# SGI-2022/Latent-Diffusion-Models-for-Shape-SDFs

Hardware: AMD Instinct MI355X
Metric: SDF queries/sec on 256^3 grid (+ DDPM sample steps/sec) (higher is better)
Workload: dtype bf16; 1 GPU; config4: decode B=64 shapes on a 256^3 grid on 1 rank (the whole grid is the one slab: no gather); batch=64, grid=256, latent_dim=256, decoder=DeepSDF 8x512 skip@4, parallelism=zslab1

## Files before the change

### latent-diffusion-models-for-shape-sdfs_amd/csrc/decoder_common.h

```cpp
#pragma once
#include "ldm_internal.h"

#include <math.h>

namespace ldm {
namespace dec {

enum DecMode { kModeGrid = 0, kModePoints = 1, kModeBricks = 2 };

#define LDM_STR2(x) #x
#define LDM_STR(x) LDM_STR2(x)

__device__ __forceinline__ float grid_axis(int i, float vs, float origin) {
#pragma clang fp contract(off)
    float t = (float)i * vs;
    return t + origin;
}

__device__ __forceinline__ void grid_point(int p, int N, int k0, float vs, float origin,
                                           float& x, float& y, float& z) {
    const int nn = N * N;
    const int k = k0 + p / nn;
    const int r = p - (p / nn) * nn;
    const int j = r / N;
    const int i = r - j * N;
    x = grid_axis(i, vs, origin);
    y = grid_axis(j, vs, origin);
    z = grid_axis(k, vs, origin);
}


template <typename T>
struct Elem;
template <>
struct Elem<__bf16> {
    static __device__ __forceinline__ unsigned pack(float a, float b) {
        typedef float f32x2 __attribute__((ext_vector_type(2)));
        const f32x2 v = {a, b};
        return __builtin_bit_cast(unsigned, __builtin_convertvector(v, bf16x2));
    }
    static __device__ __forceinline__ float round(float x) { return (float)(__bf16)x; }
    static __device__ __forceinline__ f32x16 mfma(u32x4 a, u32x4 b, f32x16 c) {
        return __builtin_amdgcn_mfma_f32_32x32x16_bf16(__builtin_bit_cast(bf16x8, a),
                                                       __builtin_bit_cast(bf16x8, b), c, 0, 0, 0);
    }
    static __device__ __forceinline__ f32x4 mfma16(u32x4 a, u32x4 b, f32x4 c) {
        return __builtin_amdgcn_mfma_f32_16x16x32_bf16(__builtin_bit_cast(bf16x8, a),
                                                       __builtin_bit_cast(bf16x8, b), c, 0, 0, 0);
    }
};
template <>
struct Elem<_Float16> {
    static __device__ __forceinline__ unsigned pack(float a, float b) {
        f16x2 v = {(_Float16)a, (_Float16)b};
        return __builtin_bit_cast(unsigned, v);
    }
    static __device__ __forceinline__ float round(float x) { return (float)(_Float16)x; }
    static __device__ __forceinline__ f32x16 mfma(u32x4 a, u32x4 b, f32x16 c) {
        return __builtin_amdgcn_mfma_f32_32x32x16_f16(__builtin_bit_cast(f16x8, a),
                                                      __builtin_bit_cast(f16x8, b), c, 0, 0, 0);
    }
    static __device__ __forceinline__ f32x4 mfma16(u32x4 a, u32x4 b, f32x4 c) {
        return __builtin_amdgcn_mfma_f32_16x16x32_f16(__builtin_bit_cast(f16x8, a),
                                                      __builtin_bit_cast(f16x8, b), c, 0, 0, 0);
    }
};


__device__ __forceinline__ unsigned relu2(unsigned v) {
    typedef short s16x2 __attribute__((ext_vector_type(2)));
    s16x2 x = __builtin_bit_cast(s16x2, v);
    const s16x2 z = {0, 0};
    x = __builtin_elementwise_max(x, z);
    return __builtin_bit_cast(unsigned, x);
}

template <typename T>
__device__ __forceinline__ void acc_to_frags(const f32x16& a, u32x4& f0, u32x4& f1) {
#pragma unroll
    for (int q = 0; q < 4; ++q) {
        f0[q] = relu2(Elem<T>::pack(a[2 * q], a[2 * q + 1]));
        f1[q] = relu2(Elem<T>::pack(a[8 + 2 * q], a[8 + 2 * q + 1]));
    }
}

}
}
```

### latent-diffusion-models-for-shape-sdfs_amd/csrc/decoder_fs.hip

```cpp
#include "decoder_common.h"

namespace ldm {
namespace {
using namespace dec;

constexpr int kFsD = 4;

constexpr int kFsStep = 2048;
constexpr int kFsAct = 33 * 4 * 1024;
constexpr int kFsRed = 4 * 4 * 64 * 4;
constexpr int kFsWl = 512 * 4;
#ifndef FS_STAMP
#define FS_STAMP 0
#endif
constexpr int kFsStamp = FS_STAMP ? 128 * 8 : 0;
#ifndef FS_ABL
#define FS_ABL 0
#endif
static_assert(FS_ABL == 0 || FS_STAMP, "ablations are diagnostic builds");
constexpr int kFsLds = kFsAct + kFsRed + kFsWl + kFsStamp;
static_assert(kFsLds <= 160 * 1024, "LDS");

__host__ __device__ constexpr int fs_nparts(int S) { return S == 256 ? 15 : 16; }
__host__ __device__ constexpr int fs_nsteps(int S) { return S == 256 ? 384 : 448; }

template <typename T>
__global__ void fs_aux_pack_kernel(const float* __restrict__ beta, const float* __restrict__ wxyz,
                                   int B, T* __restrict__ aux) {
    const int id = blockIdx.x * blockDim.x + threadIdx.x;
    if (id >= B * 4 * 4 * 2 * 64) return;
    const int lane = id & 63;
    const int i = (id >> 6) & 1;
    const int slot = (id >> 7) & 3;
    const int w = (id >> 9) & 3;
    const int b = id >> 11;
    const int li = slot >> 1;
    const int p = slot & 1;
    float v[8] = {0, 0, 0, 0, 0, 0, 0, 0};
    if (lane < 32) {
        const int f = 128 * w + 64 * p + 32 * i + lane;
        const float* wx = wxyz + ((size_t)li * kHidden + f) * 3;
        const float bb = beta[((size_t)b * 2 + li) * kHidden + f];
        const float hi = Elem<T>::round(bb);
        v[0] = wx[0]; v[1] = wx[1]; v[2] = wx[2];
        v[3] = wx[0]; v[4] = wx[1]; v[5] = wx[2];
        v[6] = hi;    v[7] = bb - hi;
    }
    T* o = aux + (size_t)id * 8;
#pragma unroll
    for (int e = 0; e < 8; ++e) o[e] = (T)v[e];
}

struct FArgs {
    const uint8_t* stream;
    const uint8_t* aux;
    const float* w_last;
    const float* xyz;
    float* out;
    float b_last;
    int npts, tiles_per_shape, n_tiles;
    int N, k0;
    float vs, origin;
    const int32_t* bricks;
    const int32_t* count;
    int nb, nbt;
};

enum FsEpi { FE_NONE = 0, FE_LATE = 1, FE_EARLY = 2, FE_FIN0 = 3, FE_FIN1 = 4 };

struct FSrc {
    bool shape;
    uint32_t off;
    bool none = false;
};

struct FCtx {
    int lane, wave, h;
    uint32_t voff;
    char* smem;
    __amdgpu_buffer_rsrc_t rw;
    __amdgpu_buffer_rsrc_t ra;
    uint32_t s_beg, s_end;
    uint32_t s_iss;
    uint32_t baux_w;
    uint32_t aux_w;
    uint32_t aux_next;
    u32x4 auxn[2];
    u32x4 ring[kFsD][2];
    u32x4 b[4];
    float part[4];
    float* out;
    int npts, prev_shape, prev_local;
    float b_last;
    unsigned long long* st;
    int st_i;
    bool st_on;
    const int32_t* bricks;
    int N, nb, nbt;
};

__device__ __forceinline__ void stamp(FCtx& c) {
    if (FS_STAMP) {
        if (c.st_on && c.lane == 0 && c.st_i < 128) c.st[c.st_i] = __builtin_readcyclecounter();
        ++c.st_i;
    }
}

__device__ __forceinline__ u32x4 bld(__amdgpu_buffer_rsrc_t r, uint32_t voff, uint32_t soff) {
    return __builtin_bit_cast(u32x4, __builtin_amdgcn_raw_buffer_load_b128(r, voff, soff, 0));
}

__device__ __forceinline__ void load_aux(FCtx& c, FSrc s) {
    if (s.none) return;
    const __amdgpu_buffer_rsrc_t r = s.shape ? c.ra : c.rw;
    c.auxn[0] = bld(r, c.voff, s.off);
    c.auxn[1] = bld(r, c.voff + 1024u, s.off);
}

__device__ __forceinline__ uint32_t opaque(uint32_t v) {
    asm volatile("" : "+v"(v));
    return v;
}

__device__ __forceinline__ int opaque_s(int v) {
    asm volatile("" : "+s"(v));
    return v;
}

__device__ __forceinline__ char* lds_at(const FCtx& c, uint32_t off) {
    return c.smem + (opaque(c.voff) + off);
}
__device__ __forceinline__ u32x4* act_w(const FCtx& c, int late) {
    return reinterpret_cast<u32x4*>(lds_at(c, (uint32_t)(late + 4 * c.wave) * 4096u));
}
__device__ __forceinline__ const f32x4* wl_at(const FCtx& c, int p, int i) {
    const uint32_t h = opaque(c.voff) >> 9;
    return reinterpret_cast<const f32x4*>(
        c.smem + kFsAct + kFsRed + (((c.wave * 2 + p) * 2 + i) * 2) * 64 + h * 64);
}

__device__ __forceinline__ float* red_w(const FCtx& c) {
    return reinterpret_cast<float*>(c.smem + kFsAct + c.wave * 4 * 64 * 4 + (opaque(c.voff) >> 2));
}

__device__ __forceinline__ void fs_bar() {
    if (FS_ABL & 4) return;
    asm volatile("s_waitcnt lgkmcnt(0)\n\ts_barrier" ::: "memory");
}

__device__ __forceinline__ void read_b(FCtx& c, int pos) {
    const u32x4* p = reinterpret_cast<const u32x4*>(lds_at(c, pos * 4096));
#pragma unroll
    for (int n = 0; n < 4; ++n) c.b[n] = p[n * 64];
}

__device__ __forceinline__ void issue(FCtx& c, int r) {
    const uint32_t so = c.s_iss + (uint32_t)(r >> 1) * 2u * kFsStep;
    const uint32_t vo = c.voff + (uint32_t)(r & 1) * kFsStep;
    if (FS_ABL & 1) return;
    c.ring[r][0] = bld(c.rw, vo, so);
    c.ring[r][1] = bld(c.rw, vo + 1024u, so);
}

__device__ __forceinline__ void next_group(FCtx& c) {
    c.s_iss += 4u * kFsStep;
    if (c.s_iss == c.s_end) c.s_iss = c.s_beg;
}

__device__ __forceinline__ float relu_f(float x) {
    return __builtin_bit_cast(float, max(__builtin_bit_cast(int, x), 0));
}

template <typename T, int EK>
__device__ __forceinline__ void epi_unit(FCtx& c, const f32x16 (&accY)[2][4], int u) {
    const int t = u >> 1, s = u & 1;
    const int i = t >> 2, n = t & 3;
    if (FS_ABL & 2) return;
    if (EK == FE_LATE || EK == FE_EARLY) {
        u32x4 f;
#pragma unroll
        for (int q = 0; q < 4; ++q)
            f[q] = relu2(Elem<T>::pack(accY[i][n][8 * s + 2 * q], accY[i][n][8 * s + 2 * q + 1]));
        u32x4* p = act_w(c, EK == FE_LATE ? 16 : 0);
        p[((2 * i + s) * 4 + n) * 64] = f;
    } else if (EK == FE_FIN0 || EK == FE_FIN1) {
        const f32x4* w = wl_at(c, EK == FE_FIN0 ? 0 : 1, i);
        float part = c.part[n];
#pragma unroll
        for (int q = 2 * s; q < 2 * s + 2; ++q) {
            const f32x4 wv = w[q];
#pragma unroll
            for (int e = 0; e < 4; ++e) part = fmaf(relu_f(accY[i][n][4 * q + e]), wv[e], part);
        }
        c.part[n] = part;
    }
}

template <typename T, int EK>
__device__ __forceinline__ void epi_step(FCtx& c, const f32x16 (&accY)[2][4], int k) {
    if (EK == FE_NONE || k == 15) return;
    epi_unit<T, EK>(c, accY, k);
    if (k == 14) epi_unit<T, EK>(c, accY, 15);
    if (EK == FE_FIN1 && k == 14) {
        float* rw = red_w(c);
#pragma unroll
        for (int n = 0; n < 4; ++n) {
            rw[n * 64] = c.part[n];
            c.part[n] = 0.f;
        }
    }
}

__device__ __forceinline__ void fin_store(const FCtx& c, int shape, int local) {
    const int lane = (int)(opaque(c.voff) >> 4);
    if (local < 0 || lane >= 32) return;
    const float* rr = reinterpret_cast<const float*>(
        c.smem + kFsAct + c.wave * 64 * 4 + (opaque(c.voff) >> 2));
    float s = 0.f;
#pragma unroll
    for (int w = 0; w < 4; ++w) s += rr[w * 4 * 64] + rr[w * 4 * 64 + 32];
    const int pt = local * kTilePoints + 32 * c.wave + lane;
    if (pt < c.npts) {
        const __amdgpu_buffer_rsrc_t ro = __builtin_amdgcn_make_buffer_rsrc(
            (void*)(c.out + (size_t)shape * c.npts), (short)0, 0x7ffffff0, 0x00020000);
        __builtin_amdgcn_raw_buffer_store_b32(__builtin_bit_cast(uint32_t, tanhf(s + c.b_last)),
                                              ro, (uint32_t)pt * 4u, 0, 2 );
    }
}

__device__ __forceinline__ int list_at(const int32_t* list, int i) {
    typedef const __attribute__((address_space(4))) int32_t* const_i32;
    return ((const_i32)(uintptr_t)list)[i];
}

__device__ __forceinline__ void brick_origin(int gid, int nb_, int& shape, int& i0, int& j0,
                                             int& k0) {
    const int nb = opaque_s(nb_);
    const int nb2 = nb * nb, nb3 = nb2 * nb;
    shape = gid / nb3;
    const int id = gid - shape * nb3;
    const int bz = id / nb2, r = id - bz * nb2;
    const int by = r / nb;
    i0 = 8 * (r - by * nb);
    j0 = 8 * by;
    k0 = 8 * bz;
}

__device__ __forceinline__ void fin_store_bricks(const FCtx& c, int tile) {
    const int lane = (int)(opaque(c.voff) >> 4);
    if (tile < 0 || lane >= 32) return;
    const float* rr = reinterpret_cast<const float*>(
        c.smem + kFsAct + c.wave * 64 * 4 + (opaque(c.voff) >> 2));
    float s = 0.f;
#pragma unroll
    for (int w = 0; w < 4; ++w) s += rr[w * 4 * 64] + rr[w * 4 * 64 + 32];
    const int gid = list_at(c.bricks, tile >> 2);
    LDM_DASSERT(gid >= 0 && gid < c.nbt);
    int shape, i0, j0, k0;
    brick_origin(gid, c.nb, shape, i0, j0, k0);
    const int idx = 128 * (tile & 3) + 32 * c.wave + lane;
    const int i = i0 + (idx & 7), j = j0 + ((idx >> 3) & 7);
    const int k = k0 + 2 * (tile & 3) + (c.wave >> 1);
    const int N = c.N;
    if ((unsigned)gid < (unsigned)c.nbt && i < N && j < N && k < N) {
        const __amdgpu_buffer_rsrc_t ro = __builtin_amdgcn_make_buffer_rsrc(
            (void*)(c.out + ((size_t)shape * N + k) * N * N), (short)0, 0x7ffffff0, 0x00020000);
        __builtin_amdgcn_raw_buffer_store_b32(__builtin_bit_cast(uint32_t, tanhf(s + c.b_last)),
                                              ro, (uint32_t)(j * N + i) * 4u, 0, 2 );
    }
}

template <int MODE>
__device__ __forceinline__ void fin_store_mode(const FCtx& c) {
    if (MODE == kModeBricks) fin_store_bricks(c, c.prev_local);
    else fin_store(c, c.prev_shape, c.prev_local);
}

__device__ __forceinline__ void valu_slot(int v) {
    if (v == 2) __builtin_amdgcn_sched_group_barrier(0x002, 2, 0);
    else if (v == 4) __builtin_amdgcn_sched_group_barrier(0x002, 4, 0);
}

template <typename T>
__device__ __forceinline__ void mfma_pair(f32x16 (&acc)[2][4], const u32x4& a0, const u32x4& a1,
                                          const u32x4& b, int n) {
    acc[0][n] = Elem<T>::mfma(a0, b, acc[0][n]);
    acc[1][n] = Elem<T>::mfma(a1, b, acc[1][n]);
}

template <typename T, int EK, int K0, int BAR>
__device__ __forceinline__ void group4(FCtx& c, f32x16 (&acc)[2][4], const f32x16 (&accY)[2][4],
                                       int p0) {
    constexpr int BP = 1;
    const char* gbase = lds_at(c, (p0 + 1) * 4096);
#pragma unroll
    for (int r = 0; r < 4; ++r) {
        const u32x4* nb = reinterpret_cast<const u32x4*>(gbase + r * 4096);
        const u32x4 a0 = c.ring[r][0], a1 = c.ring[r][1];
        const int k = K0 + r;
        const int V = (EK == FE_NONE || k == 15) ? 0 : (k == 14 ? 4 : 2);
        if (r == BAR) {
#pragma unroll
            for (int n = 0; n < BP; ++n) mfma_pair<T>(acc, a0, a1, c.b[n], n);
            for (int n = 0; n < BP; ++n) {
                __builtin_amdgcn_sched_group_barrier(0x008, 2, 0);
            }
            __builtin_amdgcn_sched_barrier(0);
            fs_bar();
            __builtin_amdgcn_sched_barrier(0);
#pragma unroll
            for (int n = 0; n < BP; ++n) c.b[n] = nb[n * 64];
#pragma unroll
            for (int n = BP; n < 4; ++n) {
                mfma_pair<T>(acc, a0, a1, c.b[n], n);
                c.b[n] = nb[n * 64];
            }
            issue(c, r);
            epi_step<T, EK>(c, accY, k);
            for (int n = 0; n < BP; ++n) __builtin_amdgcn_sched_group_barrier(0x100, 1, 0);
            for (int n = BP; n < 4; ++n) {
                __builtin_amdgcn_sched_group_barrier(0x008, 1, 0);
                valu_slot(V);
                __builtin_amdgcn_sched_group_barrier(0x008, 1, 0);
                __builtin_amdgcn_sched_group_barrier(0x100, 1, 0);
                valu_slot(V);
            }
        } else {
#pragma unroll
            for (int n = 0; n < 4; ++n) {
                mfma_pair<T>(acc, a0, a1, c.b[n], n);
                c.b[n] = nb[n * 64];
            }
            issue(c, r);
            epi_step<T, EK>(c, accY, k);
#pragma unroll
            for (int n = 0; n < 4; ++n) {
                __builtin_amdgcn_sched_group_barrier(0x008, 1, 0);
                valu_slot(V);
                __builtin_amdgcn_sched_group_barrier(0x008, 1, 0);
                __builtin_amdgcn_sched_group_barrier(0x100, 1, 0);
                valu_slot(V);
            }
        }
        __builtin_amdgcn_sched_group_barrier(0x020, 2, 0);
        __builtin_amdgcn_sched_barrier(0);
    }
    next_group(c);
}

template <typename T, int EK, bool BAR>
__device__ __forceinline__ void steps16e(FCtx& c, f32x16 (&acc)[2][4],
                                         const f32x16 (&accY)[2][4], int p0) {
    group4<T, EK, 0, -1>(c, acc, accY, p0);
    group4<T, EK, 4, -1>(c, acc, accY, p0 + 4);
    group4<T, EK, 8, -1>(c, acc, accY, p0 + 8);
    group4<T, EK, 12, BAR ? 3 : -1>(c, acc, accY, p0 + 12);
}

template <typename T>
__device__ __forceinline__ void steps_plain(FCtx& c, f32x16 (&acc)[2][4],
                                            const f32x16 (&accY)[2][4], int pos0, int j0, int j1) {
#pragma unroll 1
    for (int j = j0; j < j1; j += 4) group4<T, FE_NONE, 0, -1>(c, acc, accY, pos0 + j);
}

template <typename T, int EK, bool E16, int MODE = kModeGrid>
__device__ __forceinline__ void run_part(FCtx& c, f32x16 (&acc)[2][4], const f32x16 (&accY)[2][4],
                                         int nk, bool mid, bool endbar, FSrc naux, int pos0,
                                         bool bar0) {
    const f32x16 zero = {};
    const u32x4 a0 = c.auxn[0], a1 = c.auxn[1];
    if (nk == 0) {
#pragma unroll
        for (int n = 0; n < 4; ++n) {
            acc[0][n] = Elem<T>::mfma(a0, c.b[n], zero);
            acc[1][n] = Elem<T>::mfma(a1, c.b[n], zero);
        }
        load_aux(c, naux);
        stamp(c);
        return;
    }
    if (bar0) {
#pragma unroll
        for (int n = 0; n < 4; ++n) {
            acc[0][n] = Elem<T>::mfma(a0, c.b[n], zero);
            acc[1][n] = Elem<T>::mfma(a1, c.b[n], zero);
        }
        load_aux(c, naux);
        fs_bar();
        read_b(c, pos0);
    } else {
        const u32x4* p = reinterpret_cast<const u32x4*>(lds_at(c, pos0 * 4096));
#pragma unroll
        for (int n = 0; n < 4; ++n) {
            acc[0][n] = Elem<T>::mfma(a0, c.b[n], zero);
            acc[1][n] = Elem<T>::mfma(a1, c.b[n], zero);
            c.b[n] = p[n * 64];
        }
        load_aux(c, naux);
#pragma unroll
        for (int n = 0; n < 4; ++n) {
            __builtin_amdgcn_sched_group_barrier(0x008, 2, 0);
            __builtin_amdgcn_sched_group_barrier(0x100, 1, 0);
        }
        __builtin_amdgcn_sched_group_barrier(0x020, 2, 0);
        __builtin_amdgcn_sched_barrier(0);
    }
    stamp(c);
    if (!E16 && EK != FE_NONE) {
        if (mid || (endbar && nk == 16)) steps16e<T, EK, true>(c, acc, accY, pos0);
        else steps16e<T, EK, false>(c, acc, accY, pos0);
        if (EK == FE_FIN1) fin_store_mode<MODE>(c);
        stamp(c);
        if (endbar && nk == 32) {
            steps_plain<T>(c, acc, accY, pos0, 16, 28);
            group4<T, FE_NONE, 0, 3>(c, acc, accY, pos0 + 28);
        } else {
            steps_plain<T>(c, acc, accY, pos0, 16, nk);
        }
    } else if (E16) {
        steps_plain<T>(c, acc, accY, pos0, 0, 12);
        group4<T, FE_NONE, 0, 3>(c, acc, accY, pos0 + 12);
        stamp(c);
        if (endbar) steps16e<T, EK, true>(c, acc, accY, pos0 + 16);
        else steps16e<T, EK, false>(c, acc, accY, pos0 + 16);
    } else {
        steps_plain<T>(c, acc, accY, pos0, 0, nk < 16 ? nk : 16);
        stamp(c);
        steps_plain<T>(c, acc, accY, pos0, 16, nk);
    }
    stamp(c);
}

template <typename T, bool LATE>
__device__ __forceinline__ void acc_to_lds(FCtx& c, const f32x16 (&acc)[2][4]) {
    u32x4* p = act_w(c, LATE ? 16 : 0);
#pragma unroll
    for (int i = 0; i < 2; ++i)
#pragma unroll
        for (int n = 0; n < 4; ++n) {
            u32x4 f0, f1;
            acc_to_frags<T>(acc[i][n], f0, f1);
            p[(2 * i * 4 + n) * 64] = f0;
            p[((2 * i + 1) * 4 + n) * 64] = f1;
        }
}

template <typename T, int S, int MODE>
__global__ __launch_bounds__(256, 1) void dec_fs_kernel(FArgs a) {
    __shared__ __attribute__((aligned(16))) char smem[kFsLds];
    FCtx c;
    c.lane = threadIdx.x & 63;
    c.wave = __builtin_amdgcn_readfirstlane(threadIdx.x >> 6);
    c.h = c.lane >> 5;
    c.voff = (uint32_t)c.lane * 16u;
    c.smem = smem;
    c.out = a.out;
    c.npts = a.npts;
    c.b_last = a.b_last;
    c.prev_shape = 0;
    c.prev_local = -1;
    c.st = reinterpret_cast<unsigned long long*>(smem + kFsAct + kFsRed + kFsWl);
    c.st_i = 0;
    c.st_on = false;
    float* wl = reinterpret_cast<float*>(smem + kFsAct + kFsRed);

    for (int i = threadIdx.x; i < 512; i += 256) wl[i] = a.w_last[i];
    __syncthreads();
    const int n_tiles = MODE == kModeBricks ? 4 * min(max(a.count[0], 0), a.nbt) : a.n_tiles;
    if (MODE == kModeBricks) {
        c.bricks = a.bricks;
        c.N = a.N;
        c.nb = a.nb;
        c.nbt = a.nbt;
    }
    if ((int)blockIdx.x >= n_tiles) return;

    constexpr int NST = fs_nsteps(S);
    constexpr int NP = fs_nparts(S);
    constexpr uint32_t kFlags = 0x00020000u;
    c.rw = __builtin_amdgcn_make_buffer_rsrc((void*)a.stream, (short)0, 0x7ffffff0, kFlags);
    c.ra = __builtin_amdgcn_make_buffer_rsrc((void*)a.aux, (short)0, 0x7ffffff0, kFlags);
    c.s_beg = (uint32_t)c.wave * NST * kFsStep;
    c.s_end = c.s_beg + NST * kFsStep;
    c.s_iss = c.s_beg;
    c.baux_w = (uint32_t)(4 * NST + c.wave * NP) * kFsStep;
    auto brick_of = [&](int tile) -> int {
        return min(max(list_at(a.bricks, tile >> 2), 0), a.nbt - 1);
    };
    auto shape_aux = [&](int tile) -> uint32_t {
        if (MODE == kModeBricks) {
            const int nb = opaque_s(a.nb);
            return ((uint32_t)(brick_of(tile) / (nb * nb * nb)) * 4u + (uint32_t)c.wave) * 4u *
                   kFsStep;
        }
        return ((uint32_t)(tile / a.tiles_per_shape) * 4u + (uint32_t)c.wave) * 4u * kFsStep;
    };
    auto bias = [&](int pi) -> FSrc { return FSrc{false, c.baux_w + (uint32_t)pi * kFsStep}; };
    auto shp = [&](int slot) -> FSrc { return FSrc{true, c.aux_w + (uint32_t)slot * kFsStep}; };
    c.aux_w = shape_aux(blockIdx.x);
#pragma unroll
    for (int r = 0; r < kFsD; ++r) issue(c, r);
    next_group(c);

    f32x16 accA[2][4], accB[2][4];
#pragma unroll
    for (int i = 0; i < 2; ++i)
#pragma unroll
        for (int n = 0; n < 4; ++n) accB[i][n] = f32x16{};
#pragma unroll
    for (int n = 0; n < 4; ++n) c.part[n] = 0.f;
#pragma unroll 1
    for (int tile = blockIdx.x; tile < n_tiles; tile += gridDim.x) {
        int shape, local, bi0 = 0, bj0 = 0, bk0 = 0;
        if (MODE == kModeBricks) {
            brick_origin(brick_of(tile), a.nb, shape, bi0, bj0, bk0);
            local = tile;
        } else {
            shape = tile / a.tiles_per_shape;
            local = tile - shape * a.tiles_per_shape;
        }
        {
            const int nt = tile + (int)gridDim.x;
            c.aux_next = nt < n_tiles ? shape_aux(nt) : c.aux_w;
        }
        c.st_on = FS_STAMP && c.wave == 0 && tile == (int)blockIdx.x + (int)gridDim.x;
        c.st_i = 0;
        stamp(c);
        load_aux(c, shp(0));
        const uint32_t lv = opaque(c.voff);
        const bool hi = lv >= 512u;
#pragma unroll
        for (int n = 0; n < 4; ++n) {
            int pt = local * kTilePoints + 32 * n + (int)((lv >> 4) & 31u);
            if (pt >= a.npts) pt = a.npts - 1;
            float x, y, z;
            if (MODE == kModeBricks) {
                const int idx = 128 * (tile & 3) + 32 * n + (int)((lv >> 4) & 31u);
                const int m = a.N - 1;
                x = grid_axis(min(bi0 + (idx & 7), m), a.vs, a.origin);
                y = grid_axis(min(bj0 + ((idx >> 3) & 7), m), a.vs, a.origin);
                z = grid_axis(min(bk0 + (idx >> 6), m), a.vs, a.origin);
            } else if (MODE == kModePoints) {
                const float* qq = a.xyz + ((size_t)shape * a.npts + pt) * 3;
                x = qq[0];
                y = qq[1];
                z = qq[2];
            } else {
                grid_point(pt, opaque_s(a.N), a.k0, a.vs, a.origin, x, y, z);
            }
            const float xh = Elem<T>::round(x), yh = Elem<T>::round(y), zh = Elem<T>::round(z);
            u32x4 f;
            f[0] = hi ? 0u : Elem<T>::pack(xh, yh);
            f[1] = hi ? 0u : Elem<T>::pack(zh, x - xh);
            f[2] = hi ? 0u : Elem<T>::pack(y - yh, z - zh);
            f[3] = hi ? 0u : Elem<T>::pack(1.f, 1.f);
            reinterpret_cast<u32x4*>(lds_at(c, 32u * 4096u))[n * 64] = f;
        }
        read_b(c, 32);

        run_part<T, FE_NONE, false>(c, accA, accB, 0, false, false, shp(1), 0, false);
        acc_to_lds<T, false>(c, accA);
        stamp(c);
        run_part<T, FE_NONE, false>(c, accA, accB, 0, false, false, bias(2), 0, false);
        acc_to_lds<T, true>(c, accA);
        stamp(c);

        int pi = 2;
        run_part<T, FE_FIN1, false, MODE>(c, accA, accB, 32, true, false, bias(pi + 1), 0, true);
        run_part<T, FE_EARLY, true>(c, accB, accA, 32, true, true, bias(pi + 2), 0, false);
        pi += 2;
        constexpr int L2P = S == 256 ? 3 : 4;
#pragma unroll 1
        for (int l = 2; l < L2P; ++l, pi += 2) {
            const FSrc nx = (S == 512 && l == 3) ? shp(2) : bias(pi + 2);
            run_part<T, FE_LATE, false>(c, accA, accB, 32, true, false, bias(pi + 1), 0, false);
            run_part<T, FE_EARLY, true>(c, accB, accA, 32, true, true, nx, 0, false);
        }
        if (S == 256) {
            run_part<T, FE_LATE, false>(c, accA, accB, 32, true, false, shp(2), 0, false);
            fs_bar();
            acc_to_lds<T, true>(c, accA);
            stamp(c);
            run_part<T, FE_NONE, false>(c, accA, accB, 16, false, false, shp(3), 16, true);
            run_part<T, FE_EARLY, false>(c, accB, accA, 16, false, true, bias(pi + 3), 16,
                                             false);
            pi += 3;
        } else {
            run_part<T, FE_LATE, false>(c, accA, accB, 32, true, false, shp(3), 0, false);
            run_part<T, FE_EARLY, true>(c, accB, accA, 32, true, true, bias(pi + 2), 0, false);
            pi += 2;
        }
#pragma unroll 1
        for (int l = 5; l < 7; ++l, pi += 2) {
            run_part<T, FE_LATE, false>(c, accA, accB, 32, true, false, bias(pi + 1), 0, false);
            run_part<T, FE_EARLY, true>(c, accB, accA, 32, true, true, bias(pi + 2), 0, false);
        }
        run_part<T, FE_LATE, false>(c, accA, accB, 32, true, false, bias(pi + 1), 0, false);
        run_part<T, FE_FIN0, false>(c, accB, accA, 32, false, true, FSrc{true, 0, true}, 0,
                                        false);
        c.prev_shape = shape;
        c.prev_local = local;
        c.aux_w = c.aux_next;
    }
#pragma unroll
    for (int u = 0; u < 16; ++u) epi_unit<T, FE_FIN1>(c, accB, u);
    {
        float* rw = red_w(c);
#pragma unroll
        for (int n = 0; n < 4; ++n) rw[n * 64] = c.part[n];
    }
    fs_bar();
    fin_store_mode<MODE>(c);
    asm volatile("s_waitcnt vmcnt(0)" ::: "memory");
    if (FS_STAMP && c.wave == 0) {
        __builtin_amdgcn_s_waitcnt(0);
        for (int k = c.lane; k < 128; k += 64)
            reinterpret_cast<unsigned long long*>(a.out)[(size_t)blockIdx.x * 128 + k] = c.st[k];
    }
}

template <typename T, int S>
void launch_fs(const FArgs& a, bool points, hipStream_t s, int grid) {
    if (points)
        hipLaunchKernelGGL((dec_fs_kernel<T, S, kModePoints>), dim3(grid), dim3(256), 0, s, a);
    else
        hipLaunchKernelGGL((dec_fs_kernel<T, S, kModeGrid>), dim3(grid), dim3(256), 0, s, a);
}

template <typename T, int S>
void launch_fs_bricks(const FArgs& a, hipStream_t s, int grid) {
    hipLaunchKernelGGL((dec_fs_kernel<T, S, kModeBricks>), dim3(grid), dim3(256), 0, s, a);
}

}

size_t decoder_fs_aux_bytes(int B) { return (size_t)B * 4 * 4 * kFsStep; }

int decoder_fs_n_stages(int skip_width) { return fs_nsteps(skip_width == 253 ? 256 : 512); }

int decoder_fs_fwd(const ldm_decoder_t* w, const float* beta, const float* xyz, int B, int npts,
                   int N, int k0, float vs, float origin, float* out, void* ws, size_t ws_bytes,
                   hipStream_t s, int num_cus, const int32_t* bricks, const int32_t* count,
                   int n_bricks) {
    const int S = w->skip_width == 253 ? 256 : 512;
    LDM_REQUIRE(w->n_stages == fs_nsteps(S), LDM_EINVAL, "split layout: n_stages %d != %d",
                w->n_stages, fs_nsteps(S));
    LDM_REQUIRE(ws != nullptr && ws_bytes >= decoder_fs_aux_bytes(B) && LDM_ALIGNED(ws, 16),
                LDM_ENOSPC, "workspace too small: need %zu bytes, got %zu",
                decoder_fs_aux_bytes(B), ws_bytes);
    LDM_REQUIRE((size_t)B * 4 * 4 * kFsStep < 0x7ffffff0u, LDM_EINVAL,
                "split layout: %d shapes exceed the aux buffer range", B);
    {
        const int n = B * 4 * 4 * 2 * 64;
        if (w->dtype == LDM_BF16)
            hipLaunchKernelGGL(fs_aux_pack_kernel<__bf16>, dim3((n + 255) / 256), dim3(256), 0, s,
                               beta, w->wxyz, B, (__bf16*)ws);
        else
            hipLaunchKernelGGL(fs_aux_pack_kernel<_Float16>, dim3((n + 255) / 256), dim3(256), 0,
                               s, beta, w->wxyz, B, (_Float16*)ws);
        if (int e = launch_status("fs_aux_pack")) return e;
    }
    FArgs a;
    a.stream = (const uint8_t*)w->weights;
    a.aux = (const uint8_t*)ws;
    a.w_last = w->w_last;
    a.xyz = xyz;
    a.out = out;
    a.b_last = w->b_last;
    a.npts = npts;
    a.tiles_per_shape = (npts + kTilePoints - 1) / kTilePoints;
    a.n_tiles = B * a.tiles_per_shape;
    a.bricks = bricks;
    a.count = count;
    a.nb = (N + 7) / 8;
    a.nbt = n_bricks;
    const int mode = bricks ? kModeBricks : xyz ? kModePoints : kModeGrid;
    if (mode == kModeBricks) a.n_tiles = 4 * n_bricks;
    a.N = N;
    a.k0 = k0;
    a.vs = vs;
    a.origin = origin;
    const int grid = a.n_tiles < num_cus ? a.n_tiles : num_cus;
    if (mode != kModeBricks) {
        const bool points = mode == kModePoints;
        if (w->dtype == LDM_BF16) {
            if (S == 256) launch_fs<__bf16, 256>(a, points, s, grid);
            else launch_fs<__bf16, 512>(a, points, s, grid);
        } else {
            if (S == 256) launch_fs<_Float16, 256>(a, points, s, grid);
            else launch_fs<_Float16, 512>(a, points, s, grid);
        }
    } else if (w->dtype == LDM_BF16) {
        if (S == 256) launch_fs_bricks<__bf16, 256>(a, s, grid);
        else launch_fs_bricks<__bf16, 512>(a, s, grid);
    } else {
        if (S == 256) launch_fs_bricks<_Float16, 256>(a, s, grid);
        else launch_fs_bricks<_Float16, 512>(a, s, grid);
    }
    return launch_status("ldm_decoder_fwd(split)");
}

}
```

Before: 471.3 million queries/s.

## Pipeline layer-0 MFMAs with LDS stores and cheapen grid index division

```diff
diff --git a/latent-diffusion-models-for-shape-sdfs_amd/csrc/decoder_common.h b/latent-diffusion-models-for-shape-sdfs_amd/csrc/decoder_common.h
--- a/latent-diffusion-models-for-shape-sdfs_amd/csrc/decoder_common.h
+++ b/latent-diffusion-models-for-shape-sdfs_amd/csrc/decoder_common.h
@@ -1,4 +1,5 @@
 #pragma once
+#include "grid_index.h"
 #include "ldm_internal.h"
 
 #include <math.h>
@@ -44,6 +45,11 @@
         return __builtin_amdgcn_mfma_f32_32x32x16_bf16(__builtin_bit_cast(bf16x8, a),
                                                        __builtin_bit_cast(bf16x8, b), c, 0, 0, 0);
     }
+    static __device__ __forceinline__ f32x16 mfma_v(u32x4 a, u32x4 b) {
+        f32x16 d;
+        asm volatile("v_mfma_f32_32x32x16_bf16 %0, %1, %2, 0" : "=&v"(d) : "v"(a), "v"(b));
+        return d;
+    }
     static __device__ __forceinline__ f32x4 mfma16(u32x4 a, u32x4 b, f32x4 c) {
         return __builtin_amdgcn_mfma_f32_16x16x32_bf16(__builtin_bit_cast(bf16x8, a),
                                                        __builtin_bit_cast(bf16x8, b), c, 0, 0, 0);
@@ -59,6 +65,11 @@
     static __device__ __forceinline__ f32x16 mfma(u32x4 a, u32x4 b, f32x16 c) {
         return __builtin_amdgcn_mfma_f32_32x32x16_f16(__builtin_bit_cast(f16x8, a),
                                                       __builtin_bit_cast(f16x8, b), c, 0, 0, 0);
+    }
+    static __device__ __forceinline__ f32x16 mfma_v(u32x4 a, u32x4 b) {
+        f32x16 d;
+        asm volatile("v_mfma_f32_32x32x16_f16 %0, %1, %2, 0" : "=&v"(d) : "v"(a), "v"(b));
+        return d;
     }
     static __device__ __forceinline__ f32x4 mfma16(u32x4 a, u32x4 b, f32x4 c) {
         return __builtin_amdgcn_mfma_f32_16x16x32_f16(__builtin_bit_cast(f16x8, a),
diff --git a/latent-diffusion-models-for-shape-sdfs_amd/csrc/decoder_fs.hip b/latent-diffusion-models-for-shape-sdfs_amd/csrc/decoder_fs.hip
--- a/latent-diffusion-models-for-shape-sdfs_amd/csrc/decoder_fs.hip
+++ b/latent-diffusion-models-for-shape-sdfs_amd/csrc/decoder_fs.hip
@@ -64,6 +64,7 @@
     const int32_t* bricks;
     const int32_t* count;
     int nb, nbt;
+    GridDiv gd;
 };
 
 enum FsEpi { FE_NONE = 0, FE_LATE = 1, FE_EARLY = 2, FE_FIN0 = 3, FE_FIN1 = 4 };
@@ -171,6 +172,11 @@
     return __builtin_bit_cast(float, max(__builtin_bit_cast(int, x), 0));
 }
 
+__device__ __forceinline__ float acc_read(float a) {
+    asm volatile("" : "+a"(a));
+    return a;
+}
+
 template <typename T, int EK>
 __device__ __forceinline__ void epi_unit(FCtx& c, const f32x16 (&accY)[2][4], int u) {
     const int t = u >> 1, s = u & 1;
@@ -190,7 +196,11 @@
         for (int q = 2 * s; q < 2 * s + 2; ++q) {
             const f32x4 wv = w[q];
 #pragma unroll
-            for (int e = 0; e < 4; ++e) part = fmaf(relu_f(accY[i][n][4 * q + e]), wv[e], part);
+            for (int e = 0; e < 4; ++e) {
+                const float v = EK == FE_FIN1 ? acc_read(accY[i][n][4 * q + e])
+                                              : accY[i][n][4 * q + e];
+                part = fmaf(relu_f(v), wv[e], part);
+            }
         }
         c.part[n] = part;
     }
@@ -370,16 +380,6 @@
                                          bool bar0) {
     const f32x16 zero = {};
     const u32x4 a0 = c.auxn[0], a1 = c.auxn[1];
-    if (nk == 0) {
-#pragma unroll
-        for (int n = 0; n < 4; ++n) {
-            acc[0][n] = Elem<T>::mfma(a0, c.b[n], zero);
-            acc[1][n] = Elem<T>::mfma(a1, c.b[n], zero);
-        }
-        load_aux(c, naux);
-        stamp(c);
-        return;
-    }
     if (bar0) {
 #pragma unroll
         for (int n = 0; n < 4; ++n) {
@@ -410,7 +410,10 @@
     if (!E16 && EK != FE_NONE) {
         if (mid || (endbar && nk == 16)) steps16e<T, EK, true>(c, acc, accY, pos0);
         else steps16e<T, EK, false>(c, acc, accY, pos0);
-        if (EK == FE_FIN1) fin_store_mode<MODE>(c);
+        if (EK == FE_FIN1) {
+            stamp(c);
+            fin_store_mode<MODE>(c);
+        }
         stamp(c);
         if (endbar && nk == 32) {
             steps_plain<T>(c, acc, accY, pos0, 16, 28);
@@ -432,9 +435,9 @@
     stamp(c);
 }
 
-template <typename T, bool LATE>
+template <typename T>
 __device__ __forceinline__ void acc_to_lds(FCtx& c, const f32x16 (&acc)[2][4]) {
-    u32x4* p = act_w(c, LATE ? 16 : 0);
+    u32x4* p = act_w(c, 16);
 #pragma unroll
     for (int i = 0; i < 2; ++i)
 #pragma unroll
@@ -444,6 +447,31 @@
             p[(2 * i * 4 + n) * 64] = f0;
             p[((2 * i + 1) * 4 + n) * 64] = f1;
         }
+}
+
+template <typename T, bool LATE>
+__device__ __forceinline__ void layer0_part(FCtx& c, FSrc naux) {
+    const u32x4 a[2] = {c.auxn[0], c.auxn[1]};
+    u32x4* p = act_w(c, LATE ? 16 : 0);
+    f32x16 t[2];
+    t[0] = Elem<T>::mfma_v(a[0], c.b[0]);
+#pragma unroll
+    for (int q = 0; q < 8; ++q) {
+        const int i = q & 1, n = q >> 1;
+        if (q < 7) t[(q + 1) & 1] = Elem<T>::mfma_v(a[(q + 1) & 1], c.b[(q + 1) >> 1]);
+        if (q == 0) {
+            asm volatile("s_nop 10" : "+v"(t[0]));
+            load_aux(c, naux);
+            stamp(c);
+        }
+        __builtin_amdgcn_sched_barrier(0);
+        u32x4 f0, f1;
+        acc_to_frags<T>(t[q & 1], f0, f1);
+        p[(2 * i * 4 + n) * 64] = f0;
+        p[((2 * i + 1) * 4 + n) * 64] = f1;
+        __builtin_amdgcn_sched_barrier(0);
+    }
+    stamp(c);
 }
 
 template <typename T, int S, int MODE>
@@ -530,6 +558,17 @@
         load_aux(c, shp(0));
         const uint32_t lv = opaque(c.voff);
         const bool hi = lv >= 512u;
+        const uint32_t p0 = (uint32_t)local * kTilePoints;
+        uint32_t ti = 0, tj = 0, tk = 0;
+        if (MODE == kModeGrid) {
+            grid_first(p0, (uint32_t)a.N, a.gd, ti, tj, tk);
+            tk += (uint32_t)a.k0;
+        }
+        const float* row = nullptr;
+        if (MODE == kModePoints) {
+            row = a.xyz + (size_t)shape * a.npts * 3;
+            asm volatile("" : "+s"(row));
+        }
 #pragma unroll
         for (int n = 0; n < 4; ++n) {
             int pt = local * kTilePoints + 32 * n + (int)((lv >> 4) & 31u);
@@ -542,12 +581,18 @@
                 y = grid_axis(min(bj0 + ((idx >> 3) & 7), m), a.vs, a.origin);
                 z = grid_axis(min(bk0 + (idx >> 6), m), a.vs, a.origin);
             } else if (MODE == kModePoints) {
-                const float* qq = a.xyz + ((size_t)shape * a.npts + pt) * 3;
+                const float* qq = row + (size_t)pt * 3;
                 x = qq[0];
                 y = qq[1];
                 z = qq[2];
             } else {
-                grid_point(pt, opaque_s(a.N), a.k0, a.vs, a.origin, x, y, z);
+                const uint32_t off =
+                    grid_tail_off(p0, 32u * n + ((lv >> 4) & 31u), (uint32_t)a.npts);
+                uint32_t vi, vj, vk;
+                grid_voxel(ti, tj, tk, off, (uint32_t)a.N, a.gd.m, vi, vj, vk);
+                x = grid_axis((int)vi, a.vs, a.origin);
+                y = grid_axis((int)vj, a.vs, a.origin);
+                z = grid_axis((int)vk, a.vs, a.origin);
             }
             const float xh = Elem<T>::round(x), yh = Elem<T>::round(y), zh = Elem<T>::round(z);
             u32x4 f;
@@ -559,12 +604,8 @@
         }
         read_b(c, 32);
 
-        run_part<T, FE_NONE, false>(c, accA, accB, 0, false, false, shp(1), 0, false);
-        acc_to_lds<T, false>(c, accA);
-        stamp(c);
-        run_part<T, FE_NONE, false>(c, accA, accB, 0, false, false, bias(2), 0, false);
-        acc_to_lds<T, true>(c, accA);
-        stamp(c);
+        layer0_part<T, false>(c, shp(1));
+        layer0_part<T, true>(c, bias(2));
 
         int pi = 2;
         run_part<T, FE_FIN1, false, MODE>(c, accA, accB, 32, true, false, bias(pi + 1), 0, true);
@@ -580,7 +621,7 @@
         if (S == 256) {
             run_part<T, FE_LATE, false>(c, accA, accB, 32, true, false, shp(2), 0, false);
             fs_bar();
-            acc_to_lds<T, true>(c, accA);
+            acc_to_lds<T>(c, accA);
             stamp(c);
             run_part<T, FE_NONE, false>(c, accA, accB, 16, false, false, shp(3), 16, true);
             run_part<T, FE_EARLY, false>(c, accB, accA, 16, false, true, bias(pi + 3), 16,
@@ -681,6 +722,7 @@
     a.k0 = k0;
     a.vs = vs;
     a.origin = origin;
+    a.gd = mode == kModeGrid ? grid_div(N) : GridDiv{0, 0, 0};
     const int grid = a.n_tiles < num_cus ? a.n_tiles : num_cus;
     if (mode != kModeBricks) {
         const bool points = mode == kModePoints;
diff --git a/latent-diffusion-models-for-shape-sdfs_amd/csrc/grid_index.h b/latent-diffusion-models-for-shape-sdfs_amd/csrc/grid_index.h
--- /dev/null
+++ b/latent-diffusion-models-for-shape-sdfs_amd/csrc/grid_index.h
@@ -0,0 +1,60 @@
+#pragma once
+#include <stdint.h>
+
+#if defined(__HIPCC__) || defined(__CUDACC__)
+#define LDM_HD __host__ __device__ inline __attribute__((always_inline))
+#else
+#define LDM_HD inline
+#endif
+
+namespace ldm {
+namespace dec {
+
+struct GridDiv {
+    uint32_t m, mw, sh;
+};
+
+inline GridDiv grid_div(int N) {
+    GridDiv d;
+    d.m = (uint32_t)(((1ull << 32) + (uint32_t)N - 1) / (uint32_t)N);
+    uint32_t lg = 0;
+    while ((1u << lg) < (uint32_t)N) ++lg;
+    d.sh = 31 + lg;
+    d.mw = (uint32_t)(((1ull << d.sh) + (uint32_t)N - 1) / (uint32_t)N);
+    return d;
+}
+
+LDM_HD uint32_t grid_mulhi(uint32_t a, uint32_t b) {
+    return (uint32_t)(((uint64_t)a * b) >> 32);
+}
+
+LDM_HD uint32_t grid_mul24(uint32_t a, uint32_t b) {
+    return (a & 0xffffffu) * (b & 0xffffffu);
+}
+
+LDM_HD void grid_first(uint32_t p0, uint32_t N, GridDiv d, uint32_t& i, uint32_t& j,
+                       uint32_t& k) {
+    const uint32_t row = (uint32_t)(((uint64_t)p0 * d.mw) >> d.sh);
+    i = p0 - row * N;
+    k = grid_mulhi(row, d.m);
+    j = row - k * N;
+}
+
+LDM_HD void grid_voxel(uint32_t i0, uint32_t j0, uint32_t k0, uint32_t off, uint32_t N,
+                       uint32_t m, uint32_t& i, uint32_t& j, uint32_t& k) {
+    const uint32_t x = i0 + off;
+    const uint32_t cx = grid_mulhi(x, m);
+    i = x - grid_mul24(cx, N);
+    const uint32_t y = j0 + cx;
+    const uint32_t cy = grid_mulhi(y, m);
+    j = y - grid_mul24(cy, N);
+    k = k0 + cy;
+}
+
+LDM_HD uint32_t grid_tail_off(uint32_t p0, uint32_t want, uint32_t npts) {
+    const uint32_t last = npts - 1u - p0;
+    return want < last ? want : last;
+}
+
+}
+}
```

Measured after the change: 477.7 million queries/s, median of 6. +1.4%, better.
